# Twilight-Dream-Of-Magic/KolmogorovLike-DataCompressor

Measured on AMD Instinct MI355X. Metric: compress MB/s at fixed block size, bit-exact vs reference; 1/2/4/8-GPU scaling, higher is better.
Workload: dtype u8; 1 GPU; enwik-style synthetic text (kolm.datagen.enwik_like, seed 20251212+rank), 256 MiB per GPU resident in HBM, 1 MiB fixed blocks, candidates 0..8 + MDL, payloads emitted in HBM; block_size=1048576, bytes_per_gpu=268435456, blocks_per_gpu=256, parallelism=block-shard x1

## Files before the change

include/kolm.h:

```cpp
#ifndef KOLM_H
#define KOLM_H

#include <stddef.h>
#include <stdint.h>

#ifdef __cplusplus
extern "C" {
#endif

#define KOLM_OK 0
#define KOLM_EARG (-1)
#define KOLM_ECAP (-2)
#define KOLM_EHIP (-3)
#define KOLM_ERCCL (-4)
#define KOLM_ENOINIT (-5)
#define KOLM_EFORMAT (-6)
#define KOLM_ERANGE (-7)
#define KOLM_EVERIFY (-8)

#define KOLM_M_RAW 0
#define KOLM_M_XOR 1
#define KOLM_M_BBWT 2
#define KOLM_M_BBWT_BP 3
#define KOLM_M_BBWT_NIB 4
// ... 160 lines not shown
typedef struct kolm_read_stats {
    uint32_t ranges;
    uint32_t blocks_decoded;
    uint32_t groups;
    uint32_t compactions;
    uint64_t bytes_returned;
    uint64_t bytes_decoded;
    double ms_decode;
    double ms_gather;
} kolm_read_stats;
int kolm_reader_open(kolm_ctx* ctx, const uint8_t* container, uint64_t cn, kolm_reader** out);
int kolm_reader_close(kolm_reader* r);
int kolm_reader_info(kolm_reader* r, uint64_t* info, uint32_t* methods, uint32_t* orig_lens, uint32_t cap);
int kolm_reader_read(kolm_reader* r, const uint64_t* offs, const uint64_t* lens, uint32_t nranges, uint8_t* out,
                     uint64_t out_cap, kolm_read_stats* stats);
int kolm_reader_read_device(kolm_reader* r, const uint64_t* offs, const uint64_t* lens, uint32_t nranges,
                            void* d_out, uint64_t out_cap, kolm_read_stats* stats);

typedef struct kolm_dedup_report {
    uint32_t blocks;
    uint32_t blocks_encoded;
    uint32_t candidate_pairs;
    uint32_t collisions;
    uint64_t bytes;
    uint64_t bytes_encoded;
    double ms_hash;
    double ms_compare;
    double ms_compact;
    double ms_expand;
} kolm_dedup_report;
int kolm_ctx_set_dedup(kolm_ctx* ctx, int enable);
int kolm_set_dedup(int enable);
int kolm_ctx_dedup_report(kolm_ctx* ctx, kolm_dedup_report* rep);
int kolm_block_fingerprints_device(kolm_ctx* ctx, const void* d_data, const uint64_t* h_bounds, uint32_t nblocks,
                                   uint64_t* h_fp);
int kolm_find_duplicates_device(kolm_ctx* ctx, const void* d_data, const uint64_t* h_bounds, uint32_t nblocks,
                                uint32_t* h_rep, kolm_dedup_report* rep);
int kolm_dedup_plan(const uint32_t* lens, const uint64_t* fps, const int32_t* force_method, uint32_t nblocks,
                    uint32_t fp_bits, const uint32_t* differ, uint32_t* pairs, uint32_t* rep, uint32_t* distinct,
                    kolm_range_seg* compact, const uint64_t* distinct_off, uint64_t* payload_off,
                    kolm_range_seg* expand, uint32_t* counts);

#define KOLM_COMM_ID_BYTES 128
typedef struct kolm_comm kolm_comm;
int kolm_comm_unique_id(uint8_t* id);
int kolm_comm_init(kolm_ctx* ctx, int nranks, int rank, const uint8_t* id, kolm_comm** out);
int kolm_comm_destroy(kolm_comm* comm);
int kolm_comm_rank(kolm_comm* comm, int* rank, int* nranks);
int kolm_comm_allreduce(kolm_comm* comm, void* values, uint32_t count, int dtype, int op);
int kolm_comm_barrier(kolm_comm* comm);
int kolm_gather_payloads(kolm_comm* comm, const void* d_arena, uint64_t nbytes, const uint32_t* method,
                         const uint64_t* payload_off, uint32_t nblocks, int dst, void* d_dst, uint64_t dst_cap,
                         uint32_t dst_cap_blocks, uint64_t* rank_bytes, uint32_t* rank_blocks,
                         uint32_t* method_all, uint64_t* off_all, int async_op);
int kolm_comm_wait(kolm_comm* comm);

#ifdef __cplusplus
}
#endif
#endif
```

kolmogorovlike-datacompressor_amd/csrc/k_blocks.hip:

```cpp
#include <algorithm>
#include <cstdio>
#include <cstdlib>

#include "kolm_internal.h"

namespace kolm {

namespace {

constexpr u32 BIG = 0xFFFFFFFFu;

struct TileGeom {
    Geom geo;
    u32 tpb;
    __device__ inline bool range(u32 t, u32& lo, u32& hi, u32& b) const {
        b = t / tpb;
        const u32 k = t - b * tpb;
        lo = geo.base(b) + k * TILE;
        const u32 e = geo.end(b);
        hi = min(lo + (u32)TILE, e);
        return lo < e;
    }
};

__device__ inline u32 wave_reduce_min(u32 v) { return wave_reduce(v, OpMinU(), BIG); }
__device__ inline u32 wave_reduce_max(u32 v) { return wave_reduce(v, OpMaxU(), 0u); }

template <bool REV, bool MAX>
__device__ inline u32 wg_excl(u32 v, u32 ident, u32* sh) {
    const u32 lane = threadIdx.x & 63, w = threadIdx.x >> 6;
    u32 incl, ex;
    if (MAX) {
        incl = REV ? wave_incl_scan_rev(v, OpMaxU(), ident) : wave_incl_scan(v, OpMaxU(), ident);
    } else {
        incl = REV ? wave_incl_scan_rev(v, OpMinU(), ident) : wave_incl_scan(v, OpMinU(), ident);
    }
    ex = REV ? KOLM_DPP(ident, incl, DPP_WAVE_SHL1, 0xF) : KOLM_DPP(ident, incl, DPP_WAVE_SHR1, 0xF);
// ... 167 lines not shown
}
__device__ inline u32 bm_next(const u32* bm, const u32* sm, u32 q, u32 hi) {
    if (q >= hi) return hi;
    u32 w = q >> 5;
    u32 v = bm[w] & (0xFFFFFFFFu << (q & 31));
    if (!v) {
        const u32 wl = (hi + 31) >> 5;
        const u32 swl = (wl + 31) >> 5;
        u32 sw = (w + 1) >> 5;
        if (sw >= swl) return hi;
        u32 sv = ((w + 1) & 31) ? (sm[sw] & (0xFFFFFFFFu << ((w + 1) & 31))) : sm[sw];
        while (!sv) {
            if (++sw >= swl) return hi;
            sv = sm[sw];
        }
        w = (sw << 5) + __ffs(sv) - 1;
        if (w >= wl) return hi;
        v = bm[w];
    }
    const u32 r = (w << 5) + __ffs(v) - 1;
    return r < hi ? r : hi;
}

__device__ inline void dprof(u64* prof, u32 k, u64& last) {
    if (prof && threadIdx.x == 0) {
        const u64 now = wall_clock64();
        atomicAdd((unsigned long long*)&prof[k], (unsigned long long)(now - last));
        atomicMax((unsigned long long*)&prof[24 + k], (unsigned long long)(now - last));
        last = now;
    }
}
template <u32 NT>
__global__ __launch_bounds__(NT) void k_duval_span(Geom geo, u32 spb, const u8* s, u32* fstart, uint4* fpre,
                                                   u32* nfac, u64* prof, u32 wave_w, u32 grp) {
    constexpr u32 SPAN = DUVAL_CH * NT;
    u64 tlast = prof ? wall_clock64() : 0;
    __shared__ __align__(16) u8 t[SPAN + NT * DUVAL_PAD + 16];
    __shared__ u32 bm[SPAN / 32];
    __shared__ u32 sm[(SPAN + 1023) / 1024];
    __shared__ u32 sh[NT / 64];
    const u32 sp = blockIdx.x, tid = threadIdx.x;
    const u32 b = sp / spb, k = sp - b * spb;
    const u32 lo = geo.base(b) + k * SPAN;
    const u32 e = geo.end(b), e_blk = e;
    if (lo >= e) {
        if (tid == 0) nfac[sp] = 0;
        return;
    }
    const u32 n = min(SPAN, e - lo);
    if (n == SPAN && (lo & 15) == 0) {
        const uint4* src = reinterpret_cast<const uint4*>(s + lo);
        for (u32 i = tid; i < SPAN / 16; i += NT) {
            const uint4 v = src[i];
            u32* d = reinterpret_cast<u32*>(&t[lds_addr(i * 16)]);
            d[0] = v.x;
            d[1] = v.y;
            d[2] = v.z;
            d[3] = v.w;
        }
    } else {
        for (u32 i = tid; i < n; i += NT) t[lds_addr(i)] = s[lo + i];
    }
    for (u32 i = tid; i < SPAN / 32; i += NT) bm[i] = 0;
    __syncthreads();
    dprof(prof, 0, tlast);
    {
        const u32 clo = tid * DUVAL_CH, chi = min(clo + DUVAL_CH, n);
        u32 i = clo, j = clo + 1, kk = clo, p = 1;
// ... 263 lines not shown
}

__device__ inline Pre text_pre(const u8* s, u32 x, u32 e) {
    u32 w[8];
    if (x + 48 <= e) {
#pragma unroll
        for (u32 k = 0; k < 4; ++k) {
            const u64 v = load8u(s, x + 8 * k);
            w[2 * k] = __builtin_bswap32((u32)v);
            w[2 * k + 1] = __builtin_bswap32((u32)(v >> 32));
        }
    } else {
#pragma unroll
        for (u32 k = 0; k < 8; ++k) {
            u32 v4 = 0;
            for (u32 b = 0; b < 4; ++b) {
                const u32 y = x + 4 * k + b;
                v4 = (v4 << 8) | (y < e ? s[y] : 0u);
            }
            w[k] = v4;
        }
    }
    return Pre{make_uint4(w[0], w[1], w[2], w[3]), make_uint4(w[4], w[5], w[6], w[7])};
}

__device__ inline u32 rdl(u32 v, u32 l) { return (u32)__builtin_amdgcn_readlane((int)v, l); }
__device__ inline Pre rdl(const Pre& p, u32 l) {
    return Pre{make_uint4(rdl(p.a.x, l), rdl(p.a.y, l), rdl(p.a.z, l), rdl(p.a.w, l)),
               make_uint4(rdl(p.b.x, l), rdl(p.b.y, l), rdl(p.b.z, l), rdl(p.b.w, l))};
}

__global__ __launch_bounds__(64) void k_duval_merge(Geom geo, u32 cpb, u32 span, const u8* s, const u32* fstart,
                                                    const uint4* fpre, const u32* nfac, u32* stack, u32* fcount,
                                                    u8* flag, u64* prof) {
    __shared__ u32 lstk[MERGE_LDS];
    __shared__ Pre lpre[PRE_LDS];
    __shared__ u32 lok[PRE_LDS];
    const u64 t0 = prof ? wall_clock64() : 0;
    u32 ncmp = 0, nstep = 0, npush = 0, nmerge = 0, nlyn = 0, nb_try = 0, nb_lim = 0, nb_hit = 0;
    u32 mxs[2] = {~0u, ~0u}, mys[2] = {~0u, ~0u}, mL[2] = {0, 0};
    bool mex[2] = {false, false}, mlt[2] = {false, false};
    int mold = 0;
    u64 tlyn = 0;
    const u32 b = blockIdx.x, lane = threadIdx.x;
    const u32 base = geo.base(b), end = geo.end(b);
    u32 tot = 0;
    for (u32 k = lane; k < cpb; k += 64)
        if (base + k * span < end) tot += nfac[b * cpb + k];
    tot = wave_reduce(tot, OpAddU(), 0u);
    volatile u32* stk = tot <= MERGE_LDS ? lstk : stack + base;
    u32 sp = 0;
    u32 top = 0, tok = 0;
    Pre tpre{};
    for (u32 k = 0; k < cpb; ++k) {
        const u32 c = b * cpb + k;
        const u32 lo = base + k * span;
        if (lo >= end) break;
        const u32 hi = min(lo + span, end);
        const u32 nf = nfac[c];
        static_assert(DUVAL_PF == 64, "group 0 of the span comes from fpre");
        u32 g0 = 0;
        u32 vst = lane < nf ? fstart[lo + lane] : hi;
        u32 vnx = lane + 1 < nf ? fstart[lo + lane + 1] : hi;
        Pre vpr{};
        if (lane < nf) {
            vpr.a = fpre[((u64)c * DUVAL_PF + lane) * 2];
            vpr.b = fpre[((u64)c * DUVAL_PF + lane) * 2 + 1];
// ... 273 lines not shown
        atomicOr((unsigned long long*)&bm[wa], (unsigned long long)(ma & me));
        return;
    }
    atomicOr((unsigned long long*)&bm[wa], (unsigned long long)ma);
    for (u32 w = wa + 1; w < we; ++w) bm[w] = ~0ull;
    atomicOr((unsigned long long*)&bm[we], (unsigned long long)me);
}

__global__ __launch_bounds__(256) void k_bbwt_gather_m(Geom geo, const u32* SA, const u8* prevc, u8* out,
                                                       const u64* bm) {
    const u32 g0 = xcd_tile() * 4096u + 16u * threadIdx.x;
    if (g0 >= geo.N) return;
    u32 m = (u32)(bm[g0 >> 6] >> (g0 & 63)) & 0xFFFFu;
    while (m) {
        const u32 g = g0 + (u32)__ffs(m) - 1;
        if (g < geo.N) out[g] = prevc[SA[g]];
        m &= m - 1;
    }
}

}

u32 bbwt_early_round() { return 3u; }

void launch_mark_active(const Seg* cur, const u32* ncur_dev, u32 bound, u64* bm, hipStream_t s) {
    if (bound) k_mark_active<<<(bound + 255) / 256, 256, 0, s>>>(cur, ncur_dev, bound, bm);
}
void launch_bbwt_gather_masked(const Geom& geo, const u32* SA, const u8* prevc, u8* out, const u64* bm,
                               hipStream_t s) {
    if (!geo.N) return;
    k_bbwt_gather_m<<<(u32)((geo.N + 4095) / 4096), 256, 0, s>>>(geo, SA, prevc, out, bm);
}

u64* dprof_buf() {
    static u64* prof = nullptr;
    static const bool dp = getenv("KOLM_DUVAL_PROF") && atoi(getenv("KOLM_DUVAL_PROF"));
    if (dp && !prof) {
        KOLM_HIP_CHECK(hipMalloc(&prof, 40 * sizeof(u64)));
        KOLM_HIP_CHECK(hipMemset(prof, 0, 40 * sizeof(u64)));
    }
    return prof;
}

u32 duval_span_bytes(const Geom& geo) {
    (void)geo;
    return DUVAL_CH * 64;
}

void launch_lyndon(const Geom& geo, const u8* text, u8* flag, u8* FEd, u32* fstart, uint4* fpre, u32* nfac,
                   u32* stack, u32* fcount, u32* tile_tmp, hipStream_t s, KTimer* kt) {
    if (!geo.N) return;
    TileGeom tg{geo, (geo.bs + TILE - 1) / TILE};
    const u32 nt = tg.tpb * geo.nb;
    u32* A = tile_tmp;
    u32* B = tile_tmp + nt;
    const u32 span = duval_span_bytes(geo);
    const u32 cpb = (geo.bs + span - 1) / span;
    const u32 nch = cpb * geo.nb;
    const u64 N = geo.N;
    KOLM_HIP_CHECK(hipMemsetAsync(flag, 0, geo.N, s));
    {
        KScope k(kt, KT_LYNDON, "k_duval_span", N);
        k_duval_span<64><<<nch, 64, 0, s>>>(geo, cpb, text, fstart, fpre, nfac, dprof_buf(), DUVAL_WAVE_W, 1u);
    }
    {
        KScope k(kt, KT_LYNDON, "k_duval_merge", (u64)nch * 8);
        k_duval_merge<<<geo.nb, 64, 0, s>>>(geo, cpb, span, text, fstart, fpre, nfac, stack, fcount, flag,
                                             dprof_buf());
    }
    if (u64* prof = dprof_buf()) {
        u64 h[40];
        KOLM_HIP_CHECK(hipStreamSynchronize(s));
        KOLM_HIP_CHECK(hipMemcpy(h, prof, sizeof h, hipMemcpyDeviceToHost));
        KOLM_HIP_CHECK(hipMemset(prof, 0, 40 * sizeof(u64)));
        fprintf(stderr, "[kolm] duval_span us per workgroup (mean/max):");
        for (int k = 0; k < 11; ++k) fprintf(stderr, " %d:%.1f/%.1f", k, (double)h[k] / nch / 100.0, (double)h[24 + k] / 100.0);
        fprintf(stderr, " | merge us per block mean %.1f max %.1f, compares/block %.1f, 512-B steps/block %.1f, "
                "span factors/block %.1f\n", (double)h[11] / geo.nb / 100.0, (double)h[12] / 100.0,
                (double)h[13] / geo.nb, (double)h[14] / geo.nb, (double)h[15] / geo.nb);
        fprintf(stderr, "[kolm] merge per block: pushes %.1f merges %.1f text compares %.1f (%.1f us), final factors %.1f; "
                "batch: LCP-bounded tries %.1f, bounded %.1f, batches taken %.1f\n",
                (double)h[16] / geo.nb, (double)h[17] / geo.nb, (double)h[18] / geo.nb, (double)h[19] / geo.nb / 100.0,
                (double)h[20] / geo.nb, (double)h[21] / geo.nb, (double)h[22] / geo.nb, (double)h[23] / geo.nb);
    }
    {
        KScope k(kt, KT_LYNDON, "k_tile_starts", N);
        k_tile_starts<<<nt, WG, 0, s>>>(tg, flag, A);
        k_tiles_scan<true, false><<<geo.nb, WG, 0, s>>>(A, B, tg.tpb, BIG);
    }
    {
        KScope k(kt, KT_LYNDON, "k_fed", 2 * N);
        k_fed<<<nt, WG, 0, s>>>(tg, flag, B, FEd);
    }
}

void launch_prevc(const Geom& geo, const u8* text, const u8* flag, Factors fac, u8* prevc, hipStream_t s) {
    if (!geo.N) return;
    const u32 grid = (u32)std::min<u64>((geo.N + 255) / 256, 65535);
    if (((uintptr_t)text & 15) == 0)
        k_prevc<<<(u32)((geo.N + 4095) / 4096), 256, 0, s>>>(geo, text, flag, fac, prevc);
    else
        k_prevc1<<<grid, 256, 0, s>>>(geo, text, flag, fac, prevc);
}

void launch_bbwt_gather(const Geom& geo, const u32* SA, const u8* prevc, u8* out, hipStream_t s) {
    if (!geo.N) return;
    k_bbwt_gather<<<(u32)((geo.N + 4095) / 4096), 256, 0, s>>>(geo, SA, prevc, out);
}

}
```

kolmogorovlike-datacompressor_amd/csrc/kolm_api.cpp:

```cpp
#include <hip/hip_runtime.h>

#include <algorithm>
#include <atomic>
#include <chrono>
#include <sys/mman.h>
#include <condition_variable>
#include <cstdio>
#include <cstdlib>
#include <cstring>
#include <functional>
#include <map>
#include <memory>
#include <mutex>
#include <string>
#include <thread>
#include <vector>

#include "../../include/kolm.h"
#include "kolm_internal.h"
#include "verify_core.h"
#include "dedup_core.h"

using namespace kolm;

// ... 103 lines not shown
        (void)hipGetLastError();
        KOLM_HIP_CHECK(hipEventSynchronize(a));
        KOLM_HIP_CHECK(hipEventSynchronize(b));
        e = hipEventElapsedTime(&ms, a, b);
    }
    KOLM_HIP_CHECK(e);
    return ms;
}

struct TScope {
    kolm_ctx* c;
    int fam;
    const char* name;
    u64 bytes;
    hipEvent_t a = nullptr;
    TScope(kolm_ctx* c_, int fam_, const char* name_, u64 bytes_);
    ~TScope() noexcept(false);
};
}

struct kolm_ctx {
    int device = 0;
    hipStream_t stream = nullptr;
    hipStream_t aux = nullptr;
    hipStream_t active = nullptr;
    hipStream_t rp = nullptr;
    bool serial = false;
    bool verify = false;
    kolm_verify_report vrep{};
    u32 vshard = 0;
    bool dedup = false;
    kolm_dedup_report drep{};
    hipEvent_t evd[2] = {};
    static constexpr int NSTAGE = 4;
    u8* stage[NSTAGE] = {};
    hipEvent_t stage_ev[NSTAGE] = {};
    u8* h_res = nullptr;
    size_t h_res_cap = 0, h_res_len = 0, h_res_off = 0;
    hipStream_t up = nullptr, dl = nullptr;
    hipEvent_t up_ev = nullptr;
    std::unique_ptr<CopyPool> pool;
    hipEvent_t evj[4] = {};
    hipEvent_t evr[2] = {};
    hipEvent_t evg[2] = {};
    hipEvent_t eva = nullptr;
    std::mutex mu;
    std::map<std::string, DevBuf> bufs;
    u32* h_cnt = nullptr;
    u32* h_rt = nullptr;
    u32* d_rt = nullptr;
    u32 rt_seq = 0;
    u32* h_tail = nullptr;
    size_t h_tail_cap = 0;
    u32* tail_host(size_t words) {
        if (words > h_tail_cap) {
            if (h_tail) KOLM_HIP_CHECK(hipHostFree(h_tail));
            h_tail = nullptr;
            h_tail_cap = 0;
            const size_t cap = std::max<size_t>(words + (words >> 2), 4096);
            KOLM_HIP_CHECK(hipHostMalloc((void**)&h_tail, cap * sizeof(u32), hipHostMallocDefault));
            h_tail_cap = cap;
        }
        return h_tail;
    }
    hipEvent_t ev[8] = {};
    bool timing = false;
// ... 464 lines not shown
                els += h[C_CLSE + k];
                segs += h[C_CLS + k];
            }
            if (!segs) continue;
            TScope t(c, KOLM_KT_SMALLSORT, w32 ? "k_small_sort_all<u32>" : "k_small_sort_all<u64>", els * 16 + segs * 8);
            launch_small_sorts(sc, w32 != 0, a, L, s);
        }
        if (h[C_EQ]) {
            TScope t(c, KOLM_KT_SMALLSORT, "k_finalize_eq", (u64)h[C_EQ] * TILE * 8);
            launch_finalize_eq(L.eq, h[C_EQ], a, L, s);
        }
        if (cyclic) pend_done = (int)round;
        round_done(round);
        ncur = (u32)std::min<u64>(h[C_ACTIVE] / 2 + geo.nb, N / 2 + geo.nb);
        ncur_dev = L.next_cnt;
        std::swap(cur, nxt);
    }
    if (pend_done >= 0) launch_update_done(blk_done, blk_last, a.blk_split, geo.nb, (u32)pend_done, s);
    if (cyclic) launch_rounds_sum(blk_last, geo.nb, c->get<u64>("rsum", 1), s);
    return out;
}

struct Pipeline {
    kolm_ctx* c;
    Geom geo;
    const u8* text;
    kolm_stats st{};
    float t_sa = 0, t_lz = 0, t_ent = 0, t_emit = 0;

    void lyndon() {
        const u64 N = geo.N;
        const u64 ntiles = (u64)((geo.bs + TILE - 1) / TILE) * geo.nb + 16;
        const u64 nch = (geo.bs + duval_span_bytes(geo) - 1) / duval_span_bytes(geo) * (u64)geo.nb + 1;
        launch_lyndon(geo, text, c->get<u8>("flag", N), c->get<u8>("FEd", N),
                      c->get<u32>("lyn_fstart", N), c->get<uint4>("lyn_fpre", nch * 128),
                      c->get<u32>("lyn_nfac", nch), c->get<u32>("lyn_stack", N), c->get<u32>("lyn_fcount", geo.nb + 1), c->get<u32>("lyn_t1", 2 * ntiles + 16),
                      c->active, c->kt());
    }
    Factors factors() { return Factors{c->get<u32>("lyn_stack", geo.N), c->get<u32>("lyn_fcount", geo.nb + 1)}; }
    hipEvent_t prevc_ready = nullptr;
    void prevc() {
        const u64 N = geo.N;
        TScope t(c, KOLM_KT_LYNDON, "k_prevc", N * 3);
        launch_prevc(geo, text, c->get<u8>("flag", N), factors(), c->get<u8>("prevc", N), c->active);
    }
    bool early_gather = false;
    hipEvent_t alpha_ready = nullptr;
    u8* cyclic(const std::function<void()>& after_round0 = {}, u8* out = nullptr) {
        const u64 N = geo.N;
        if (!out) out = c->get<u8>("bbwt", N);
        u8* prevc = c->get<u8>("prevc", N);
        u32* SA = c->get<u32>("SA", N);
        const u32 er = early_gather && prevc_ready ? bbwt_early_round() : 0u;
        bool early = false;
        const RoundHook hook = [&](u32 round, const Seg* cur, u32 bound, const u32* ncur_dev) {
            if (early || round != er) return;
            hipStream_t s = c->active, x = c->rp;
            u64* bm = c->get<u64>("bbwt_bm", (N + 63) / 64);
            KOLM_HIP_CHECK(hipMemsetAsync(bm, 0, sizeof(u64) * ((N + 63) / 64), s));
            launch_mark_active(cur, ncur_dev, bound, bm, s);
            KOLM_HIP_CHECK(hipEventRecord(c->evg[0], s));
            KOLM_HIP_CHECK(hipStreamWaitEvent(x, c->evg[0], 0));
            KOLM_HIP_CHECK(hipStreamWaitEvent(x, prevc_ready, 0));
            c->active = x;
            {
                TScope t(c, KOLM_KT_LYNDON, "k_bbwt_gather (early)", N * 6);
                launch_bbwt_gather(geo, SA, prevc, out, x);
            }
            KOLM_HIP_CHECK(hipEventRecord(c->evg[1], x));
            c->active = s;
// ... 2211 lines not shown
    }
    const u32 vs = geom_var_shift(hb.data(), nb);
    geom_init_var(geo, hb.data(), nb, c->get<u32>("dd_vb", (u64)nb + 1), c->get<u32>("dd_vmap", ((u64)hb[nb] >> vs) + 2), vs,
                  c->stream);
    return KOLM_OK;
}

}

extern "C" {

int kolm_ctx_set_dedup(kolm_ctx* c, int enable) {
    if (!c) return KOLM_EARG;
    std::lock_guard<std::mutex> g(c->mu);
    c->dedup = enable != 0;
    return KOLM_OK;
}

int kolm_set_dedup(int enable) {
    kolm_ctx* c = need_default();
    if (!c) return KOLM_ENOINIT;
    return kolm_ctx_set_dedup(c, enable);
}

int kolm_ctx_dedup_report(kolm_ctx* c, kolm_dedup_report* rep) {
    if (!c) c = need_default();
    if (!c) return KOLM_ENOINIT;
    if (!rep) return KOLM_EARG;
    std::lock_guard<std::mutex> g(c->mu);
    *rep = c->drep;
    return KOLM_OK;
}

int kolm_block_fingerprints_device(kolm_ctx* c, const void* d_data, const uint64_t* h_bounds, uint32_t nblocks,
                                   uint64_t* h_fp) {
    if (!c) return KOLM_EARG;
    if (nblocks == 0) return KOLM_OK;
    if (!d_data || !h_bounds || !h_fp) return KOLM_EARG;
    return guarded([&] {
        std::lock_guard<std::mutex> g(c->mu);
        KOLM_HIP_CHECK(hipSetDevice(c->device));
        std::vector<u32> hb, lens;
        Geom geo;
        if (int e = dedup_geom(c, h_bounds, nblocks, hb, lens, geo)) return e;
        for (auto& e : c->evd)
            if (!e) KOLM_HIP_CHECK(hipEventCreate(&e));
        c->active = c->stream;
        c->timing_reset();
        std::vector<u64> fp;
        kolm_dedup_report r{};
        dedup_fingerprints(c, static_cast<const u8*>(d_data), geo, lens, fp, r);
        dedup_collect(c);
        std::memcpy(h_fp, fp.data(), sizeof(u64) * fp.size());
        return KOLM_OK;
    });
}

int kolm_find_duplicates_device(kolm_ctx* c, const void* d_data, const uint64_t* h_bounds, uint32_t nblocks,
                                uint32_t* h_rep, kolm_dedup_report* rep) {
    if (!c) return KOLM_EARG;
    kolm_dedup_report r{};
    if (rep) *rep = r;
    if (nblocks == 0) return KOLM_OK;
    if (!d_data || !h_bounds || !h_rep) return KOLM_EARG;
    int rc = guarded([&] {
        std::lock_guard<std::mutex> g(c->mu);
// ... 370 lines not shown
```

kolmogorovlike-datacompressor_amd/csrc/kolm_internal.h:

```cpp
#pragma once
#include <hip/hip_runtime.h>
#include <stdint.h>

#include <string>

namespace kolm {

void set_err(const std::string& s);

using u8 = uint8_t;
using u16 = uint16_t;
using u32 = uint32_t;
using u64 = uint64_t;

constexpr int TILE = 2048;
constexpr int WG = 256;
constexpr int PER_THREAD = TILE / WG;
constexpr int NCLASS = 12;
constexpr u32 NONE = 0xFFFFFFFFu;
constexpr int LZ_WINDOW = 4096;
constexpr int LZ_MIN = 3;
constexpr int LZ_CAP = 32;
constexpr int MTF_CHUNK = 1024;
constexpr u32 NCAND = 11;
// ... 225 lines not shown
    const Seg* segs[NCLASS];
    u32 count[NCLASS];
    u32 wg0[NCLASS + 1];
};
void launch_keygen_small(KgClasses kc, const SortArgs& a, hipStream_t s);
void launch_keygen_large(const LTile* tiles, u32 ntiles, const LSeg* segs, const SortArgs& a,
                         hipStream_t s);
constexpr u32 MED_T = 8192;
void launch_med_sort(const LSeg* segs, u32 nseg, const u32* ndev, const SortArgs& a, const Lists& L,
                     hipStream_t s);
void launch_msd_hist(const LTile* tiles, u32 ntiles, const u32* ndev, const LSeg* segs, const SortArgs& a,
                     u32 shift, u32 width, u32* hist, hipStream_t s);
void launch_msd_scan(const LSeg* segs, u32 nseg, const u32* ndev, const SortArgs& a, u32 width, u32* hist,
                     bool last_level, const Lists& L, const Level& next, hipStream_t s);
void launch_msd_scatter(const LTile* tiles, u32 ntiles, const u32* ndev, const LSeg* segs, const SortArgs& a,
                        u32 shift, u32 width, const u32* hist, hipStream_t s);
void launch_copy_back(const LTile* tiles, u32 ntiles, const u32* ndev, const LSeg* segs, const SortArgs& a,
                      hipStream_t s);
constexpr int TINY_C = 5;
void launch_tiny_sort(int c, const Seg* segs, u32 count, const SortArgs& a, const Lists& L, hipStream_t s);
void launch_small_sort(int c, const Seg* segs, u32 count, const SortArgs& a, const Lists& L,
                       hipStream_t s);
struct SsClasses {
    const Seg* segs[NCLASS];
    u32 count[NCLASS];
    u32 wg0[NCLASS + 1];
};
void launch_small_sorts(SsClasses sc, bool w32, const SortArgs& a, const Lists& L, hipStream_t s);
void launch_finalize_eq(const Seg* eq, u32 count, const SortArgs& a, const Lists& L, hipStream_t s);
void launch_rounds_sum(const u32* blk_last, u32 nb, u64* out, hipStream_t s);
void launch_update_done(u32* blk_done, u32* blk_last, const u32* blk_split, u32 nb, u32 round, hipStream_t s);

u32 duval_span_bytes(const Geom& geo);
void launch_lyndon(const Geom& geo, const u8* text, u8* flag, u8* FEd, u32* fstart, uint4* fpre, u32* nfac,
                   u32* stack, u32* fcount, u32* tile_tmp, hipStream_t s, KTimer* kt = nullptr);
void launch_prevc(const Geom& geo, const u8* text, const u8* flag, Factors fac, u8* prevc, hipStream_t s);
void launch_bbwt_gather(const Geom& geo, const u32* SA, const u8* prevc, u8* out, hipStream_t s);
u32 bbwt_early_round();
void launch_mark_active(const Seg* cur, const u32* ncur_dev, u32 bound, u64* bm, hipStream_t s);
void launch_bbwt_gather_masked(const Geom& geo, const u32* SA, const u8* prevc, u8* out, const u64* bm,
                               hipStream_t s);

u32 lsd_tiles(const Geom& geo);
struct R0Bufs {
    const u8* text;
    const u8* FEd;
    Factors fac;
    const u8* code;
    u32 chars;
    u32 w;
    u32* KP;
    u32* K2;
    u32* SA;
    u32* K22;
    u32* SA2;
    u32* RK;
    u32* hist;
    u32 *tmax, *tmin, *cmax, *cmin;
    u32* HF;
    u32* swc = nullptr;
    u64* rec[2] = {nullptr, nullptr};
    const u16* cw = nullptr;
};
u32 launch_alpha(const Geom& geo, const u8* text, u32* pres, u8* code, u32* d_w, u32* h_w, bool compact,
                 hipStream_t s, KTimer* kt = nullptr);
void launch_alpha_async(const Geom& geo, const u8* text, u32* pres, u8* code, u16* cw, u32* d_w, u32* h_w,
                        hipStream_t s, KTimer* kt = nullptr, bool zeroed = false);
u32 alpha_width(u32 h_w);
// ... 244 lines not shown
```

kolmogorovlike-datacompressor_amd/kolm/_lib.py:

```python
from __future__ import annotations

import contextlib
import ctypes
import os
import sys
import threading
import time

import numpy as np

HERE = os.path.dirname(os.path.abspath(__file__))
LIB_PATH = os.environ.get("KOLM_LIB") or os.path.join(HERE, "libkolm_hip.so")

KOLM_NCAND = 11
KOLM_DEFAULT_MASK = 0x3FF
KOLM_FULL_MASK = 0x7FF
KOLM_HOTPATH_MASK = 0x1FF
KOLM_REPAIR_MAX_BLOCK = 1 << 22
KOLM_EFORMAT = -6
KOLM_ERANGE = -7
KOLM_EVERIFY = -8
ERRORS = {-1: "bad argument", -2: "capacity too small", -3: "HIP error", -4: "collective error",
          -5: "not initialised", -6: "malformed container", -7: "field overflow",
          -8: "payload does not decode to its input"}
# ... 152 lines not shown
    ("kolm_ctx_kernel_times", I32, [P, P, SZ, ctypes.POINTER(SZ)]),
    ("kolm_encode_blocks_device", I32, [P, P, U64, U32, U32, P, P, U64, P, P, P, P]),
    ("kolm_encode_blocks_device_var", I32, [P, P, P, U32, U32, P, P, U64, P, P, P, P]),
    ("kolm_cdc_boundaries", I32, [U8P, U64, U32, U32, U32, I32, P, U64, ctypes.POINTER(U64)]),
    ("kolm_cdc_boundaries_device", I32, [P, P, U64, U32, U32, U32, I32, P, U64, ctypes.POINTER(U64)]),
    ("kolm_decode_blocks", I32, [P, P, P, P, U32, P, U64]),
    ("kolm_decode_blocks_device", I32, [P, P, P, P, P, U32, P, U64, ctypes.POINTER(ctypes.c_double)]),
    ("kolm_compress_fixed", I32, [P, U64, U32, U32, ctypes.POINTER(P), ctypes.POINTER(U64), P]),
    ("kolm_result_copy", I32, [P, U64]),
    ("kolm_toc_write", I32, [I32, U32, U64, U32, P, P, P, P, U64, ctypes.POINTER(U64)]),
    ("kolm_toc_read", I32, [U8P, U64, P, ctypes.POINTER(U64), P, P, P, U32]),
    ("kolm_comm_unique_id", I32, [P]),
    ("kolm_comm_init", I32, [P, I32, I32, U8P, ctypes.POINTER(P)]),
    ("kolm_comm_destroy", I32, [P]),
    ("kolm_comm_rank", I32, [P, ctypes.POINTER(I32), ctypes.POINTER(I32)]),
    ("kolm_comm_allreduce", I32, [P, P, U32, I32, I32]),
    ("kolm_comm_barrier", I32, [P]),
    ("kolm_gather_payloads", I32, [P, P, U64, P, P, U32, I32, P, U64, U32, P, P, P, P, I32]),
    ("kolm_comm_wait", I32, [P]),
    ("kolm_verify_blocks_device", I32, [P, P, P, U32, P, P, P, P, ctypes.POINTER(VerifyReport)]),
    ("kolm_verify_container", I32, [P, U64, P, U64, P, U32, ctypes.POINTER(VerifyReport)]),
    ("kolm_ctx_set_verify", I32, [P, I32]),
    ("kolm_set_verify", I32, [I32]),
    ("kolm_ctx_verify_report", I32, [P, ctypes.POINTER(VerifyReport)]),
    ("kolm_range_plan", I32, [P, U32, P, P, U32, U64, P, P, P, P, P, P, P]),
    ("kolm_reader_open", I32, [P, P, U64, ctypes.POINTER(P)]),
    ("kolm_reader_close", I32, [P]),
    ("kolm_reader_info", I32, [P, P, P, P, U32]),
    ("kolm_reader_read", I32, [P, P, P, U32, P, U64, ctypes.POINTER(ReadStats)]),
    ("kolm_reader_read_device", I32, [P, P, P, U32, P, U64, ctypes.POINTER(ReadStats)]),
    ("kolm_ctx_set_dedup", I32, [P, I32]),
    ("kolm_set_dedup", I32, [I32]),
    ("kolm_ctx_dedup_report", I32, [P, ctypes.POINTER(DedupReport)]),
    ("kolm_block_fingerprints_device", I32, [P, P, P, U32, P]),
    ("kolm_find_duplicates_device", I32, [P, P, P, U32, P, ctypes.POINTER(DedupReport)]),
    ("kolm_dedup_plan", I32, [P, P, P, U32, U32, P, P, P, P, P, P, P, P, P]),
]
KOLM_COMM_ID_BYTES = 128
KOLM_ECAP = -2
KOLM_ERCCL = -4
KOLM_DECODE_MASK = 0x7FF


def decode_blocks(payloads, methods, orig_lens) -> bytes:
    ensure_init()
    nb = len(payloads)
    if nb == 0:
        return b""
    off = np.zeros(nb + 1, dtype=np.uint64)
    off[1:] = np.cumsum([len(p) for p in payloads])
    arena = np.frombuffer(b"".join(payloads) + b"\0", dtype=np.uint8)
    meth = np.ascontiguousarray(np.asarray(methods, dtype=np.uint32))
    lens = np.ascontiguousarray(np.asarray(orig_lens, dtype=np.uint32))
    total = int(lens.astype(np.uint64).sum())
    out = np.zeros(max(total, 1), dtype=np.uint8)
    check(load().kolm_decode_blocks(arena.ctypes.data, off.ctypes.data, meth.ctypes.data, lens.ctypes.data, nb,
                                    out.ctypes.data, total))
    return out[:total].tobytes()


def load():
    global _lib
    with _lock:
        if _lib is None:
            if not os.path.exists(LIB_PATH):
                raise KolmUnavailable(
# ... 42 lines not shown
        if self.verify:
            if not self.locked:
                _result_lock.acquire()
            rc = self._set(1)
            if rc:
                if not self.locked:
                    _result_lock.release()
                check(rc)
        return self

    def __exit__(self, et, ev, tb):
        global _last_verify
        if self.verify:
            try:
                if et is None or isinstance(ev, KolmVerifyError):
                    _last_verify = verify_report(self.ctx)
                self._set(1 if _ENV_VERIFY else 0)
            finally:
                if not self.locked:
                    _result_lock.release()
        return False


def last_verify() -> dict:
    return dict(_last_verify)


def dedup_report(ctx=None) -> dict:
    rep = DedupReport()
    rc = load().kolm_ctx_dedup_report(ctx, ctypes.byref(rep))
    if rc:
        raise KolmError(rc, "kolm_ctx_dedup_report")
    return rep.as_dict()


_last_dedup: dict = {}
_ENV_DEDUP = os.environ.get("KOLM_DEDUP", "0").strip() not in ("", "0")


class _dedup_scope:

    def __init__(self, ctx=None):
        self.ctx = ctx

    def _set(self, on: int) -> int:
        L = load()
        return L.kolm_set_dedup(on) if self.ctx is None else L.kolm_ctx_set_dedup(self.ctx, on)

    def __enter__(self):
        check(self._set(1))
        return self

    def __exit__(self, et, ev, tb):
        global _last_dedup
        if et is None or isinstance(ev, KolmVerifyError):
            _last_dedup = dedup_report(self.ctx)
        self._set(1 if _ENV_DEDUP else 0)
        return False


@contextlib.contextmanager
def _encode_scope(verify: bool, dedup: bool, locked: bool = False, ctx=None):
    global _last_dedup
    dedup = bool(dedup) or _ENV_DEDUP
    if not dedup:
        _last_dedup = {}
# ... 557 lines not shown
```

Baseline: 8336 MB/s.

## Add fast Lyndon factorization path via prefix-min candidates with Duval fallback

Adds a new Lyndon factorization fast path. Per-tile 8-byte prefix minima are computed and min-scanned across each block to find candidate Lyndon factor starts, and the candidates are resolved with a bounded LCP suffix-comparison scan in LDS. Blocks whose candidate count or LCP exceeds a cap are marked for fallback. The existing Duval span/merge kernels now early-exit for accepted blocks, avoiding the serial stack-merge cost, at the price of extra kernel launches and a fallback risk on repetitive data. A report API exposes how many blocks were accepted.

```diff
diff --git a/include/kolm.h b/include/kolm.h
--- a/include/kolm.h
+++ b/include/kolm.h
@@ -216,6 +216,7 @@
 int kolm_ctx_set_dedup(kolm_ctx* ctx, int enable);
 int kolm_set_dedup(int enable);
 int kolm_ctx_dedup_report(kolm_ctx* ctx, kolm_dedup_report* rep);
+int kolm_ctx_lyndon_report(kolm_ctx* ctx, uint32_t* accepted, uint32_t* fallback);
 int kolm_block_fingerprints_device(kolm_ctx* ctx, const void* d_data, const uint64_t* h_bounds, uint32_t nblocks,
                                    uint64_t* h_fp);
 int kolm_find_duplicates_device(kolm_ctx* ctx, const void* d_data, const uint64_t* h_bounds, uint32_t nblocks,
diff --git a/kolmogorovlike-datacompressor_amd/csrc/k_blocks.hip b/kolmogorovlike-datacompressor_amd/csrc/k_blocks.hip
--- a/kolmogorovlike-datacompressor_amd/csrc/k_blocks.hip
+++ b/kolmogorovlike-datacompressor_amd/csrc/k_blocks.hip
@@ -3,6 +3,7 @@
 #include <cstdlib>
 
 #include "kolm_internal.h"
+#include "lyndon_core.h"
 
 namespace kolm {
 
@@ -236,8 +237,9 @@
 }
 template <u32 NT>
 __global__ __launch_bounds__(NT) void k_duval_span(Geom geo, u32 spb, const u8* s, u32* fstart, uint4* fpre,
-                                                   u32* nfac, u64* prof, u32 wave_w, u32 grp) {
+                                                   u32* nfac, u64* prof, u32 wave_w, u32 grp, const u32* route) {
     constexpr u32 SPAN = DUVAL_CH * NT;
+    if (route && route[blockIdx.x / spb] == lyn::ACCEPT) return;
     u64 tlast = prof ? wall_clock64() : 0;
     __shared__ __align__(16) u8 t[SPAN + NT * DUVAL_PAD + 16];
     __shared__ u32 bm[SPAN / 32];
@@ -567,7 +569,8 @@
 
 __global__ __launch_bounds__(64) void k_duval_merge(Geom geo, u32 cpb, u32 span, const u8* s, const u32* fstart,
                                                     const uint4* fpre, const u32* nfac, u32* stack, u32* fcount,
-                                                    u8* flag, u64* prof) {
+                                                    u8* flag, u64* prof, const u32* route) {
+    if (route && route[blockIdx.x] == lyn::ACCEPT) return;
     __shared__ u32 lstk[MERGE_LDS];
     __shared__ Pre lpre[PRE_LDS];
     __shared__ u32 lok[PRE_LDS];
@@ -907,6 +910,211 @@
     k_bbwt_gather_m<<<(u32)((geo.N + 4095) / 4096), 256, 0, s>>>(geo, SA, prevc, out, bm);
 }
 
+namespace {
+
+struct LynReader {
+    const u8* t;
+    __device__ inline u32 amod() const { return (u32)((uintptr_t)t & 15u); }
+    __device__ inline u32 b(u32 i) const { return t[i]; }
+    __device__ inline u32 d(u32 i) const { return *reinterpret_cast<const u32*>(t + i); }
+    __device__ inline void q(u32 i, u32 e[4]) const {
+        const uint4 v = *reinterpret_cast<const uint4*>(t + i);
+        e[0] = v.x;
+        e[1] = v.y;
+        e[2] = v.z;
+        e[3] = v.w;
+    }
+};
+
+static_assert(lyn::THREADS == WG, "one lane per 16 positions of a 4 KiB tile");
+
+__device__ inline void lyn_lane(const Geom& geo, u32 tpb, u32 t, u32& b, u32& base, u32& end, u32& p, u32& n) {
+    b = t / tpb;
+    const u32 k = t - b * tpb;
+    base = geo.base(b);
+    end = geo.end(b);
+    const u64 p64 = (u64)base + (u64)k * lyn::TILE + threadIdx.x * lyn::PER;
+    p = p64 < end ? (u32)p64 : end;
+    n = min(lyn::PER, end - p);
+}
+
+__device__ inline u64 wave_min64(u64 v) {
+#pragma unroll
+    for (int o = 32; o > 0; o >>= 1) v = lyn::min64(v, (u64)__shfl_xor((unsigned long long)v, o));
+    return v;
+}
+
+__device__ inline u32 wg_scan_min64(u64 v, u64 (*sh)[WG]) {
+    const u32 tid = threadIdx.x;
+    u32 cur = 0;
+    sh[0][tid] = v;
+    __syncthreads();
+    for (u32 d = 1; d < WG; d <<= 1) {
+        u64 x = sh[cur][tid];
+        if (tid >= d) x = lyn::min64(x, sh[cur][tid - d]);
+        sh[cur ^ 1][tid] = x;
+        __syncthreads();
+        cur ^= 1;
+    }
+    return cur;
+}
+
+__global__ __launch_bounds__(WG) void k_lyn_min(Geom geo, u32 tpb, const u8* text, u64* tmin) {
+    __shared__ u64 sh[WG / 64];
+    u32 b, base, end, p, n;
+    lyn_lane(geo, tpb, blockIdx.x, b, base, end, p, n);
+    u64 m = lyn::W_MAX;
+    if (n) {
+        u32 E[6];
+        lyn::load24(LynReader{text}, p, base, end, E);
+        m = lyn::lane_min(E, n);
+    }
+    m = wave_min64(m);
+    if ((threadIdx.x & 63) == 0) sh[threadIdx.x >> 6] = m;
+    __syncthreads();
+    if (threadIdx.x == 0) tmin[blockIdx.x] = lyn::min64(lyn::min64(sh[0], sh[1]), lyn::min64(sh[2], sh[3]));
+}
+
+__global__ __launch_bounds__(WG) void k_lyn_scan(const u64* tmin, u64* tin, u32 tpb, u32* route, u32* ccount) {
+    __shared__ u64 sh[2][WG];
+    const u32 b = blockIdx.x, tid = threadIdx.x;
+    u64 carry = lyn::W_MAX;
+    for (u32 c0 = 0; c0 < tpb; c0 += WG) {
+        const u32 k = c0 + tid;
+        const u64 v = k < tpb ? tmin[(u64)b * tpb + k] : lyn::W_MAX;
+        const u32 cur = wg_scan_min64(v, sh);
+        const u64 ex = tid ? sh[cur][tid - 1] : lyn::W_MAX;
+        if (k < tpb) tin[(u64)b * tpb + k] = lyn::min64(carry, ex);
+        carry = lyn::min64(carry, sh[cur][WG - 1]);
+        __syncthreads();
+    }
+    if (tid == 0) {
+        route[b] = lyn::ACCEPT;
+        ccount[b] = 0;
+    }
+}
+
+__global__ __launch_bounds__(WG) void k_lyn_cand(Geom geo, u32 tpb, const u8* text, const u64* tmin, const u64* tin,
+                                                 u32 cap, u32* route, u32* ccount, u32* cand) {
+    __shared__ u64 sh[2][WG];
+    __shared__ u32 wsum[WG / 64];
+    __shared__ u32 gbase;
+    const u32 t = blockIdx.x, tid = threadIdx.x;
+    const u64 in = tin[t];
+    if (tmin[t] > in) return;
+    u32 b, base, end, p, n;
+    lyn_lane(geo, tpb, t, b, base, end, p, n);
+    u32 E[6] = {0, 0, 0, 0, 0, 0};
+    u64 m = lyn::W_MAX;
+    if (n) {
+        lyn::load24(LynReader{text}, p, base, end, E);
+        m = lyn::lane_min(E, n);
+    }
+    const u32 cur = wg_scan_min64(m, sh);
+    const u64 run = lyn::min64(in, tid ? sh[cur][tid - 1] : lyn::W_MAX);
+    const u32 mask = n ? lyn::lane_cands(E, n, run) : 0u;
+    const u32 cnt = (u32)__popc(mask);
+    const u32 incl = wave_incl_scan(cnt, OpAddU(), 0u);
+    if ((tid & 63) == 63) wsum[tid >> 6] = incl;
+    __syncthreads();
+    u32 off = incl - cnt, total = 0;
+    for (u32 w = 0; w < WG / 64; ++w) {
+        if (w < (tid >> 6)) off += wsum[w];
+        total += wsum[w];
+    }
+    if (total == 0) return;
+    if (tid == 0) {
+        const u32 g = atomicAdd(&ccount[b], total);
+        if (g + total > cap) atomicExch(&route[b], lyn::FALLBACK);
+        gbase = g;
+    }
+    __syncthreads();
+    u32 idx = gbase + off;
+    for (u32 i = 0; i < lyn::PER; ++i)
+        if (mask >> i & 1) {
+            if (idx < cap) cand[base + idx] = p + i;
+            ++idx;
+        }
+}
+
+__global__ __launch_bounds__(WG) void k_lyn_resolve(Geom geo, const u8* text, u32 cap, u32 lcp_cap, u32* route,
+                                                    const u32* ccount, const u32* cand, u32* stack, u32* fcount,
+                                                    u8* flag) {
+    __shared__ u32 S[lyn::CAND_MAX], A[lyn::CAND_MAX], B[lyn::CAND_MAX];
+    __shared__ u32 wsum[WG / 64];
+    __shared__ u32 fb;
+    const u32 b = blockIdx.x, tid = threadIdx.x;
+    const u32 n = ccount[b];
+    if (n > cap || route[b] != lyn::ACCEPT) {
+        if (tid == 0) route[b] = lyn::FALLBACK;
+        return;
+    }
+    const u32 base = geo.base(b), end = geo.end(b);
+    const LynReader rd{text};
+    for (u32 i = tid; i < n; i += WG) A[i] = cand[base + i];
+    if (tid == 0) fb = 0;
+    __syncthreads();
+    for (u32 i = tid; i < n; i += WG) {
+        const u32 v = A[i];
+        u32 r = 0;
+        for (u32 j = 0; j < n; ++j) r += A[j] < v;
+        S[r] = v;
+        B[r] = v;
+    }
+    __syncthreads();
+    u32* in = B;
+    u32* out = A;
+    for (u32 d = 1; d < n; d <<= 1) {
+        for (u32 i = tid; i < n; i += WG) {
+            u32 lcp;
+            bool over;
+            out[i] = lyn::scan_step(rd, in, i, d, base, end, lcp_cap, lcp, over);
+            if (over) fb = 1;
+        }
+        __syncthreads();
+        u32* x = in;
+        in = out;
+        out = x;
+    }
+    if (fb) {
+        if (tid == 0) route[b] = lyn::FALLBACK;
+        return;
+    }
+    constexpr u32 PT = lyn::CAND_MAX / WG;
+    u32 cnt = 0;
+    for (u32 e = 0; e < PT; ++e) {
+        const u32 i = tid * PT + e;
+        if (i < n && in[i] == S[i]) ++cnt;
+    }
+    const u32 incl = wave_incl_scan(cnt, OpAddU(), 0u);
+    if ((tid & 63) == 63) wsum[tid >> 6] = incl;
+    __syncthreads();
+    u32 off = incl - cnt, total = 0;
+    for (u32 w = 0; w < WG / 64; ++w) {
+        if (w < (tid >> 6)) off += wsum[w];
+        total += wsum[w];
+    }
+    for (u32 e = 0; e < PT; ++e) {
+        const u32 i = tid * PT + e;
+        if (i < n && in[i] == S[i]) {
+            stack[base + off++] = S[i];
+            flag[S[i]] = 1;
+        }
+    }
+    if (tid == 0) fcount[b] = total;
+}
+
+}
+
+bool lyn_fast_mode() {
+    if (const char* e = getenv("KOLM_LYN_FAST")) return atoi(e) != 0;
+    return true;
+}
+static u32 lyn_env(const char* name, u32 dflt, u32 lo, u32 hi) {
+    if (const char* e = getenv(name)) return (u32)std::min<u64>(hi, std::max<u64>(lo, strtoull(e, nullptr, 10)));
+    return dflt;
+}
+
 u64* dprof_buf() {
     static u64* prof = nullptr;
     static const bool dp = getenv("KOLM_DUVAL_PROF") && atoi(getenv("KOLM_DUVAL_PROF"));
@@ -921,10 +1129,11 @@
     (void)geo;
     return DUVAL_CH * 64;
 }
-
-void launch_lyndon(const Geom& geo, const u8* text, u8* flag, u8* FEd, u32* fstart, uint4* fpre, u32* nfac,
-                   u32* stack, u32* fcount, u32* tile_tmp, hipStream_t s, KTimer* kt) {
-    if (!geo.N) return;
+u32 lyn_tiles_per_block(const Geom& geo) { return (geo.bs + lyn::TILE - 1) / lyn::TILE; }
+
+bool launch_lyndon(const Geom& geo, const u8* text, u8* flag, u8* FEd, u32* fstart, uint4* fpre, u32* nfac,
+                   u32* stack, u32* fcount, u32* tile_tmp, u64* lyn_tmp, u32* lyn_route, hipStream_t s, KTimer* kt) {
+    if (!geo.N) return false;
     TileGeom tg{geo, (geo.bs + TILE - 1) / TILE};
     const u32 nt = tg.tpb * geo.nb;
     u32* A = tile_tmp;
@@ -934,14 +1143,38 @@
     const u32 nch = cpb * geo.nb;
     const u64 N = geo.N;
     KOLM_HIP_CHECK(hipMemsetAsync(flag, 0, geo.N, s));
+    const bool fast = lyn_fast_mode();
+    const u32* route = nullptr;
+    if (fast) {
+        const u32 ltpb = lyn_tiles_per_block(geo), lnt = ltpb * geo.nb;
+        const u32 cap = lyn_env("KOLM_LYN_CAND_MAX", lyn::CAND_MAX, 1, lyn::CAND_MAX);
+        const u32 lcp_cap = lyn_env("KOLM_LYN_LCP_MAX", lyn::LCP_MAX, 0, lyn::LCP_LIMIT);
+        u64* tmin = lyn_tmp;
+        u64* tin = lyn_tmp + lnt;
+        u32* ccount = lyn_route + geo.nb;
+        {
+            KScope k(kt, KT_LYNDON, "k_lyn_min", N);
+            k_lyn_min<<<lnt, WG, 0, s>>>(geo, ltpb, text, tmin);
+        }
+        {
+            KScope k(kt, KT_LYNDON, "k_lyn_cand", (u64)lnt * 32);
+            k_lyn_scan<<<geo.nb, WG, 0, s>>>(tmin, tin, ltpb, lyn_route, ccount);
+            k_lyn_cand<<<lnt, WG, 0, s>>>(geo, ltpb, text, tmin, tin, cap, lyn_route, ccount, fstart);
+        }
+        {
+            KScope k(kt, KT_LYNDON, "k_lyn_resolve", (u64)geo.nb * 8);
+            k_lyn_resolve<<<geo.nb, WG, 0, s>>>(geo, text, cap, lcp_cap, lyn_route, ccount, fstart, stack, fcount, flag);
+        }
+        route = lyn_route;
+    }
     {
         KScope k(kt, KT_LYNDON, "k_duval_span", N);
-        k_duval_span<64><<<nch, 64, 0, s>>>(geo, cpb, text, fstart, fpre, nfac, dprof_buf(), DUVAL_WAVE_W, 1u);
+        k_duval_span<64><<<nch, 64, 0, s>>>(geo, cpb, text, fstart, fpre, nfac, dprof_buf(), DUVAL_WAVE_W, 1u, route);
     }
     {
         KScope k(kt, KT_LYNDON, "k_duval_merge", (u64)nch * 8);
         k_duval_merge<<<geo.nb, 64, 0, s>>>(geo, cpb, span, text, fstart, fpre, nfac, stack, fcount, flag,
-                                             dprof_buf());
+                                             dprof_buf(), route);
     }
     if (u64* prof = dprof_buf()) {
         u64 h[40];
@@ -967,6 +1200,7 @@
         KScope k(kt, KT_LYNDON, "k_fed", 2 * N);
         k_fed<<<nt, WG, 0, s>>>(tg, flag, B, FEd);
     }
+    return fast;
 }
 
 void launch_prevc(const Geom& geo, const u8* text, const u8* flag, Factors fac, u8* prevc, hipStream_t s) {
diff --git a/kolmogorovlike-datacompressor_amd/csrc/kolm_api.cpp b/kolmogorovlike-datacompressor_amd/csrc/kolm_api.cpp
--- a/kolmogorovlike-datacompressor_amd/csrc/kolm_api.cpp
+++ b/kolmogorovlike-datacompressor_amd/csrc/kolm_api.cpp
@@ -159,6 +159,9 @@
     bool dedup = false;
     kolm_dedup_report drep{};
     hipEvent_t evd[2] = {};
+    u32 lyn_nb = 0;
+    bool lyn_fast = false;
+    hipStream_t lyn_stream = nullptr;
     static constexpr int NSTAGE = 4;
     u8* stage[NSTAGE] = {};
     hipEvent_t stage_ev[NSTAGE] = {};
@@ -689,10 +692,13 @@
         const u64 N = geo.N;
         const u64 ntiles = (u64)((geo.bs + TILE - 1) / TILE) * geo.nb + 16;
         const u64 nch = (geo.bs + duval_span_bytes(geo) - 1) / duval_span_bytes(geo) * (u64)geo.nb + 1;
-        launch_lyndon(geo, text, c->get<u8>("flag", N), c->get<u8>("FEd", N),
+        c->lyn_fast = launch_lyndon(geo, text, c->get<u8>("flag", N), c->get<u8>("FEd", N),
                       c->get<u32>("lyn_fstart", N), c->get<uint4>("lyn_fpre", nch * 128),
                       c->get<u32>("lyn_nfac", nch), c->get<u32>("lyn_stack", N), c->get<u32>("lyn_fcount", geo.nb + 1), c->get<u32>("lyn_t1", 2 * ntiles + 16),
-                      c->active, c->kt());
+                      c->get<u64>("lyn_tmin", 2 * (u64)lyn_tiles_per_block(geo) * geo.nb + 2),
+                      c->get<u32>("lyn_route", 2 * (u64)geo.nb + 2), c->active, c->kt());
+        c->lyn_nb = geo.nb;
+        c->lyn_stream = c->active;
     }
     Factors factors() { return Factors{c->get<u32>("lyn_stack", geo.N), c->get<u32>("lyn_fcount", geo.nb + 1)}; }
     hipEvent_t prevc_ready = nullptr;
@@ -2970,6 +2976,28 @@
     return KOLM_OK;
 }
 
+int kolm_ctx_lyndon_report(kolm_ctx* c, uint32_t* accepted, uint32_t* fallback) {
+    if (!c) c = need_default();
+    if (!c) return KOLM_ENOINIT;
+    if (!accepted || !fallback) return KOLM_EARG;
+    return guarded([&] {
+        std::lock_guard<std::mutex> g(c->mu);
+        *accepted = 0;
+        *fallback = c->lyn_nb;
+        if (!c->lyn_nb || !c->lyn_fast) return KOLM_OK;
+        KOLM_HIP_CHECK(hipSetDevice(c->device));
+        KOLM_HIP_CHECK(hipStreamSynchronize(c->lyn_stream));
+        std::vector<u32> route(c->lyn_nb);
+        KOLM_HIP_CHECK(hipMemcpy(route.data(), c->get<u32>("lyn_route", 2 * (u64)c->lyn_nb + 2), c->lyn_nb * sizeof(u32),
+                                 hipMemcpyDeviceToHost));
+        u32 acc = 0;
+        for (u32 r : route) acc += r == 0;
+        *accepted = acc;
+        *fallback = c->lyn_nb - acc;
+        return KOLM_OK;
+    });
+}
+
 int kolm_block_fingerprints_device(kolm_ctx* c, const void* d_data, const uint64_t* h_bounds, uint32_t nblocks,
                                    uint64_t* h_fp) {
     if (!c) return KOLM_EARG;
diff --git a/kolmogorovlike-datacompressor_amd/csrc/kolm_internal.h b/kolmogorovlike-datacompressor_amd/csrc/kolm_internal.h
--- a/kolmogorovlike-datacompressor_amd/csrc/kolm_internal.h
+++ b/kolmogorovlike-datacompressor_amd/csrc/kolm_internal.h
@@ -281,8 +281,10 @@
 void launch_update_done(u32* blk_done, u32* blk_last, const u32* blk_split, u32 nb, u32 round, hipStream_t s);
 
 u32 duval_span_bytes(const Geom& geo);
-void launch_lyndon(const Geom& geo, const u8* text, u8* flag, u8* FEd, u32* fstart, uint4* fpre, u32* nfac,
-                   u32* stack, u32* fcount, u32* tile_tmp, hipStream_t s, KTimer* kt = nullptr);
+u32 lyn_tiles_per_block(const Geom& geo);
+bool launch_lyndon(const Geom& geo, const u8* text, u8* flag, u8* FEd, u32* fstart, uint4* fpre, u32* nfac,
+                   u32* stack, u32* fcount, u32* tile_tmp, u64* lyn_tmp, u32* lyn_route, hipStream_t s,
+                   KTimer* kt = nullptr);
 void launch_prevc(const Geom& geo, const u8* text, const u8* flag, Factors fac, u8* prevc, hipStream_t s);
 void launch_bbwt_gather(const Geom& geo, const u32* SA, const u8* prevc, u8* out, hipStream_t s);
 u32 bbwt_early_round();
diff --git a/kolmogorovlike-datacompressor_amd/csrc/lyndon_core.h b/kolmogorovlike-datacompressor_amd/csrc/lyndon_core.h
--- /dev/null
+++ b/kolmogorovlike-datacompressor_amd/csrc/lyndon_core.h
@@ -0,0 +1,145 @@
+#pragma once
+#include <cstdint>
+
+#if defined(__HIPCC__)
+#define LYN_HD __host__ __device__ inline
+#else
+#define LYN_HD inline
+#endif
+#if defined(__clang__)
+#define LYN_UNROLL _Pragma("unroll")
+#else
+#define LYN_UNROLL
+#endif
+
+namespace lyn {
+
+typedef uint8_t u8;
+typedef uint32_t u32;
+typedef uint64_t u64;
+
+constexpr u32 THREADS = 256;
+constexpr u32 PER = 16;
+constexpr u32 TILE = THREADS * PER;
+constexpr u32 CAND_MAX = 1024;
+constexpr u32 LCP_MAX = 512;
+constexpr u32 LCP_LIMIT = 1u << 16;
+constexpr u64 W_MAX = ~0ull;
+constexpr u32 ACCEPT = 0, FALLBACK = 1;
+
+LYN_HD u64 min64(u64 a, u64 b) { return a < b ? a : b; }
+
+template <class R>
+LYN_HD void load24(const R& rd, u32 p, u32 base, u32 end, u32 E[6]) {
+    const u32 a = (rd.amod() + p) & 15u;
+    u32 e[6];
+    if (a == 0 && end - p >= 24) {
+        rd.q(p, e);
+        e[4] = rd.d(p + 16);
+        e[5] = rd.d(p + 20);
+    } else {
+        const u32 sh = a & 3u;
+        if (p - base >= sh && end - (p - sh) >= 28) {
+            u32 d[7];
+LYN_UNROLL
+            for (u32 k = 0; k < 7; ++k) d[k] = rd.d(p - sh + 4 * k);
+LYN_UNROLL
+            for (u32 k = 0; k < 6; ++k) e[k] = sh ? (d[k] >> (8 * sh)) | (d[k + 1] << (32 - 8 * sh)) : d[k];
+        } else {
+LYN_UNROLL
+            for (u32 k = 0; k < 6; ++k) {
+                u32 v = 0;
+                for (u32 j = 0; j < 4; ++j) {
+                    const u32 i = p + 4 * k + j;
+                    if (i < end) v |= rd.b(i) << (8 * j);
+                }
+                e[k] = v;
+            }
+        }
+    }
+LYN_UNROLL
+    for (u32 k = 0; k < 6; ++k) E[k] = __builtin_bswap32(e[k]);
+}
+
+LYN_HD u64 word_of(const u32 E[6], u32 i) {
+    const u32 k = i >> 2, r = i & 3u;
+    const u64 hi = ((u64)E[k] << 32) | E[k + 1];
+    return r ? (hi << (8 * r)) | (E[k + 2] >> (32 - 8 * r)) : hi;
+}
+
+LYN_HD u64 lane_min(const u32 E[6], u32 n) {
+    u64 m = W_MAX;
+LYN_UNROLL
+    for (u32 i = 0; i < PER; ++i)
+        if (i < n) m = min64(m, word_of(E, i));
+    return m;
+}
+
+LYN_HD u32 lane_cands(const u32 E[6], u32 n, u64 run) {
+    u32 mask = 0;
+LYN_UNROLL
+    for (u32 i = 0; i < PER; ++i) {
+        if (i < n) {
+            const u64 w = word_of(E, i);
+            if (w <= run) mask |= 1u << i;
+            run = min64(run, w);
+        }
+    }
+    return mask;
+}
+
+template <class R>
+LYN_HD u64 word_at(const R& rd, u32 p, u32 base, u32 end) {
+    if (p < end && end - p >= 8) {
+        const u32 sh = (rd.amod() + p) & 3u;
+        if (sh == 0) return ((u64)__builtin_bswap32(rd.d(p)) << 32) | __builtin_bswap32(rd.d(p + 4));
+        if (p - base >= sh && end - (p - sh) >= 12) {
+            const u32 d0 = rd.d(p - sh), d1 = rd.d(p - sh + 4), d2 = rd.d(p - sh + 8);
+            const u32 e0 = (d0 >> (8 * sh)) | (d1 << (32 - 8 * sh)), e1 = (d1 >> (8 * sh)) | (d2 << (32 - 8 * sh));
+            return ((u64)__builtin_bswap32(e0) << 32) | __builtin_bswap32(e1);
+        }
+    }
+    u64 w = 0;
+    for (u32 j = 0; j < 8; ++j) w = (w << 8) | (p + j < end ? (u64)rd.b(p + j) : 0ull);
+    return w;
+}
+
+template <class R>
+LYN_HD bool suffix_less(const R& rd, u32 x, u32 y, u32 base, u32 end, u32 lcp_cap, u32& lcp, bool& over) {
+    const bool sw = x > y;
+    const u32 lo = sw ? y : x, hi = sw ? x : y;
+    bool lo_less = false;
+    over = false;
+    for (u32 l = 0;; l += 8) {
+        if (l > lcp_cap) {
+            lcp = l;
+            over = true;
+            return false;
+        }
+        const u64 wa = word_at(rd, lo + l, base, end), wb = word_at(rd, hi + l, base, end);
+        if (wa != wb) {
+            lcp = l + (u32)__builtin_clzll(wa ^ wb) / 8;
+            lo_less = wa < wb;
+            break;
+        }
+        if (end - hi <= l + 8) {
+            lcp = end - hi;
+            break;
+        }
+    }
+    over = lcp > lcp_cap;
+    return sw ? !lo_less : lo_less;
+}
+
+template <class R>
+LYN_HD u32 scan_step(const R& rd, const u32* in, u32 i, u32 d, u32 base, u32 end, u32 lcp_cap, u32& lcp, bool& over) {
+    const u32 a = in[i];
+    over = false;
+    lcp = 0;
+    if (i < d) return a;
+    const u32 b = in[i - d];
+    if (a == b) return a;
+    return suffix_less(rd, b, a, base, end, lcp_cap, lcp, over) ? b : a;
+}
+
+}
diff --git a/kolmogorovlike-datacompressor_amd/kolm/_lib.py b/kolmogorovlike-datacompressor_amd/kolm/_lib.py
--- a/kolmogorovlike-datacompressor_amd/kolm/_lib.py
+++ b/kolmogorovlike-datacompressor_amd/kolm/_lib.py
@@ -208,6 +208,7 @@
     ("kolm_ctx_set_dedup", I32, [P, I32]),
     ("kolm_set_dedup", I32, [I32]),
     ("kolm_ctx_dedup_report", I32, [P, ctypes.POINTER(DedupReport)]),
+    ("kolm_ctx_lyndon_report", I32, [P, ctypes.POINTER(U32), ctypes.POINTER(U32)]),
     ("kolm_block_fingerprints_device", I32, [P, P, P, U32, P]),
     ("kolm_find_duplicates_device", I32, [P, P, P, U32, P, ctypes.POINTER(DedupReport)]),
     ("kolm_dedup_plan", I32, [P, P, P, U32, U32, P, P, P, P, P, P, P, P, P]),
@@ -316,6 +317,14 @@
     if rc:
         raise KolmError(rc, "kolm_ctx_dedup_report")
     return rep.as_dict()
+
+
+def lyndon_report(ctx=None) -> dict:
+    acc, fb = U32(0), U32(0)
+    rc = load().kolm_ctx_lyndon_report(ctx, ctypes.byref(acc), ctypes.byref(fb))
+    if rc:
+        raise KolmError(rc, "kolm_ctx_lyndon_report")
+    return {"accepted": int(acc.value), "fallback": int(fb.value)}
 
 
 _last_dedup: dict = {}
```

New measurement: 8821 MB/s (median of 6 runs). 5.8% higher.
